# haowenz/FEM

Measured on AMD Instinct MI355X. Metric: mapped Mreads/s (100 bp, e=3) at 1/2/4/8 MI355X + achieved HBM GB/s vs roofline, higher is better.
Workload: dtype u32/u64 integer + 32-bit Myers bit-vectors

## Files before the change

fem_amd/csrc/fem_seed_join.hip.h:

```cpp
#pragma once
#include "fem_seed_dense.hip.h"

namespace femk {

#ifndef FEM_JOIN_SLOTS_HI
#define FEM_JOIN_SLOTS_HI 32768u
#endif
#ifndef FEM_JOIN_OPT
#define FEM_JOIN_OPT 15
#endif
#ifndef FEM_JOIN_OPT_HI
#define FEM_JOIN_OPT_HI 12
#endif
#ifndef FEM_JOIN_ABL
#define FEM_JOIN_ABL 0
#endif
#ifndef FEM_JOIN_SLOTS_LO
#define FEM_JOIN_SLOTS_LO 32768u
#endif
constexpr uint32_t join_slots(int R, bool padded = false) { return R >= 7 ? FEM_JOIN_SLOTS_HI : padded ? FEM_JOIN_SLOTS_LO : 32768u; }
#ifndef FEM_JOIN_BATCH_HI
#define FEM_JOIN_BATCH_HI 3
#endif

#ifndef FEM_JOIN_SPLIT_MAX_R
#define FEM_JOIN_SPLIT_MAX_R 10
#endif
#ifndef FEM_JOIN_BATCH_FULL
#define FEM_JOIN_BATCH_FULL 2
#endif

constexpr uint32_t join_bitmap_words(int R, bool padded = false) { return join_slots(R, padded) / 32u + 4u; }

__device__ __forceinline__ uint32_t lanes_below(uint64_t m) {
  return __builtin_amdgcn_mbcnt_hi((uint32_t)(m >> 32), __builtin_amdgcn_mbcnt_lo((uint32_t)m, 0u));
}

__device__ __forceinline__ void lds_or(uint32_t *w, uint32_t bits) {
  (void)__hip_atomic_fetch_or(w, bits, __ATOMIC_RELAXED, __HIP_MEMORY_SCOPE_WAVEFRONT);
}

template <int R, bool BANKED = false, bool PADDED = false>
__device__ bool join_read(const SeedParams &p, uint32_t s_start, uint32_t s_lo, uint32_t s_freq, uint32_t *bitmap,
                          uint32_t *flg , uint32_t *scatter ,
                          uint32_t *cand_lds, uint32_t &kept0, uint32_t &kept1, uint32_t seq_base = 0u ) {
  const uint32_t ln = lane_id();
  constexpr uint32_t kSlots = join_slots(R, PADDED);
  constexpr uint32_t kSlotBits = kSlots == 65536u ? 16u : kSlots == 32768u ? 15u : 14u;
  static_assert(kSlots == (1u << kSlotBits), "a power of two of slots: 16, 32 or 64 Ki");
  constexpr uint32_t kWordBits = kSlotBits - 5u;
  constexpr uint32_t kWords = kSlots / 32u;
  constexpr uint32_t kPeriodBits = kSlotBits + 3u;
  constexpr uint32_t kFlagCap = dense_flag_cap(R);
  constexpr int kOpt = R <= 6 ? FEM_JOIN_OPT : FEM_JOIN_OPT_HI;
  constexpr bool kOptPairs = (kOpt & 1) != 0, kOptSent = (kOpt & 2) != 0 || (PADDED && R <= 6), kOptLong = (kOpt & 4) != 0, kOptHit = (kOpt & 8) != 0;
  constexpr bool kSecondProbe = true;
  constexpr uint32_t kProbeMin = kOptPairs ? 16u : 8u;
  constexpr uint32_t kFlgStride = kFlagCap + 1u;
  constexpr uint32_t kUnits = 2u * (uint32_t)kStep;
  const uint32_t e = (uint32_t)p.e;
  const uint32_t *occ32 = p.occ32;
  kept0 = 0, kept1 = 0;
  if (__builtin_amdgcn_ballot_w64(s_freq > kDenseMaxList)) return false;
  auto pack_sf = [&](uint32_t start, uint32_t freq) -> uint32_t {
    const uint32_t f_c = freq < (uint32_t)kWave ? freq : (uint32_t)kWave;
    return start | (freq << 16) | ((f_c - (freq != 0u ? 1u : 0u)) << 26);
  };
  const uint32_t s_sf = pack_sf(s_start, s_freq);
  const uint64_t s_addr = (uint64_t)(uintptr_t)(occ32 + s_lo);
  const uint32_t s_alo = (uint32_t)s_addr, s_ahi = (uint32_t)(s_addr >> 32);
  uint32_t lane4 = ln * 4u;
  if (PADDED) asm("" : "+v"(lane4));
  const uint32_t sent_a = 0xF0000000u + ln * 2304u, sent_b = 0xF0000000u + 149504u + (ln << 8);
  static_assert(PADDED || (64u * 2304u + 2048u == 149504u && 149504u + 64u * 256u + 2048u < (1u << kPeriodBits)), "sentinel families inside one period");
  const uint64_t q_is1 = __builtin_amdgcn_ballot_w64((ln >> 2) == 1u), q_is2 = __builtin_amdgcn_ballot_w64((ln >> 2) == 2u),
                 q_is3 = __builtin_amdgcn_ballot_w64((ln >> 2) == 3u);
  uint32_t nxt[R], nxt_sf[R];
  typedef const __attribute__((address_space(1))) uint8_t *GlobalBytes;
  auto run_base_of = [&](uint32_t alo, uint32_t ahi, uint32_t lane) -> GlobalBytes {
    const uint64_t a = (uint64_t)(uint32_t)__builtin_amdgcn_readlane((int)alo, (int)lane) |
                       ((uint64_t)(uint32_t)__builtin_amdgcn_readlane((int)ahi, (int)lane) << 32);
    return (GlobalBytes)(uintptr_t)a;
  };
  auto run_base = [&](uint32_t lane) -> GlobalBytes { return run_base_of(s_alo, s_ahi, lane); };
  auto prefetch_of = [&](uint32_t sf, uint32_t alo, uint32_t ahi, uint32_t u) {
    GlobalBytes base[R];
#pragma unroll
    for (int t = 0; t < R; ++t) {
      nxt_sf[t] = (uint32_t)__builtin_amdgcn_readlane((int)sf, (int)(u * R + t));
      base[t] = run_base_of(alo, ahi, u * R + t);
    }
    if (PADDED) asm volatile("" : "+v"(lane4));
#pragma unroll
    for (int t = 0; t < R; ++t) {
      const uint32_t last4 = nxt_sf[t] >> 24;
      if (PADDED)
        nxt[t] = *(const __attribute__((address_space(1))) uint32_t *)(base[t] + lane4);
      else
        nxt[t] = *(const __attribute__((address_space(1))) uint32_t *)(base[t] + (lane4 < last4 ? lane4 : last4));
    }
  };
  auto prefetch = [&](uint32_t u) { prefetch_of(s_sf, s_alo, s_ahi, u); };
  auto insert = [&](uint32_t v) -> uint32_t {
    const bool valid = v < kDenseVLimit;
    const uint32_t bit = valid ? 1u << ((v >> 3) & 31u) : 0u;
    const uint32_t widx = valid ? __builtin_amdgcn_ubfe(v, 8u, kWordBits) : ln;
    return lds_or_rtn(bitmap + widx, bit) & bit;
  };
  auto word_of = [&](uint32_t x, uint32_t from) -> uint32_t * {
    uint32_t idx = __builtin_amdgcn_ubfe(x, from, kWordBits);
    asm("" : "+v"(idx));
    return bitmap + idx;
  };
  auto insert_plain = [&](uint32_t v) -> uint32_t {
    const uint32_t bit = 1u << ((v >> 3) & 31u);
    return lds_or_rtn(word_of(v, 8u), bit) & bit;
  };
  auto mark = [&](uint32_t v, uint32_t hit) {
    if (FEM_JOIN_ABL & 4) {
      asm volatile("" ::"v"(hit));
      return;
    }
    if (hit) {
      const uint32_t qm = (v >> 3) - 1u, qp = (v >> 3) + 1u;
      lds_or(word_of(qm, 5u), 1u << (qm & 31u));
      lds_or(word_of(qp, 5u), 1u << (qp & 31u));
    }
  };
  auto window = [&](uint32_t v) -> uint32_t {
    const uint32_t qm = (v >> 3) - 1u;
    const uint32_t *w = word_of(qm, 5u);
    return __builtin_amdgcn_alignbit(w[1], w[0], qm & 31u);
  };
  constexpr uint32_t kNearTop = 0x60000000u;
  auto window_top = [&](uint32_t v) -> uint32_t {
    const uint32_t qs = (v >> 3) - 30u;
    const uint32_t *w = word_of(qs, 5u);
    return __builtin_amdgcn_alignbit(w[1], w[0], qs & 31u);
  };
  prefetch(0);
  uint32_t cmin = 0xFFFFFFFFu, cmax = 0u;
  uint32_t surv_groups = 0;
  bool any_hi = false;
#pragma unroll 1
  for (uint32_t u = 0; u < kUnits; ++u) {
    const uint32_t g = u >= (uint32_t)kStep ? u - (uint32_t)kStep : u;
    uint32_t f[R], st[R];
    uint32_t n_g = 0, f_max = 0;
    auto smax = [](uint32_t a_, uint32_t b_) -> uint32_t {
      uint32_t m;
      asm("s_max_u32 %0, %1, %2" : "=s"(m) : "s"(a_), "s"(b_) : "scc");
      return m;
    };
    const bool keep_all = BANKED && (nxt_sf[R - 1] & kSelKeepAll) != 0u;
#pragma unroll
    for (int t = 0; t < R; ++t) {
      const uint32_t sf = nxt_sf[t];
      f[t] = (sf >> 16) & 0xFFu, st[t] = sf & (BANKED ? kSelKeepAll - 1u : 0xFFFFu);
      n_g += f[t];
      f_max = t == 0 ? f[0] : smax(f[t], f_max);
    }
    uint32_t val[R];
#pragma unroll
    for (int t = 0; t < R; ++t) val[t] = nxt[t];
    if (u + 1u < kUnits) prefetch(u + 1u);
    const bool skip = (FEM_JOIN_ABL & 32) || n_g <= (uint32_t)p.a || (n_g == f[R - 1] && !keep_all);
    uint32_t n_flag = 0;
    uint32_t *flg_g = flg + g * kFlgStride;
    if (kOptPairs) {
      flg_g[ln] = 0xFFFFFFFFu;
      if (kFlagCap > (uint32_t)kWave) flg_g[ln + (uint32_t)kWave] = 0xFFFFFFFFu;
    }
    if (!skip) {
      uint32_t first_max = val[0];
#pragma unroll
      for (int t = 1; t < R; ++t) first_max = val[t] > first_max ? val[t] : first_max;
      const bool plain = f_max <= (uint32_t)kWave && __builtin_amdgcn_ballot_w64(first_max >= kDenseRemap) == 0;
      if (R <= FEM_JOIN_SPLIT_MAX_R && plain) {
#define FEM_JOIN_UNIT_PLAIN true
#include "fem_seed_join_unit.hip.h"
#undef FEM_JOIN_UNIT_PLAIN
      } else {
#define FEM_JOIN_UNIT_PLAIN false
#include "fem_seed_join_unit.hip.h"
#undef FEM_JOIN_UNIT_PLAIN
      }
    }
    if (kSecondProbe && n_flag > kProbeMin) {
      const bool have0 = ln < n_flag, have1 = ln + (uint32_t)kWave < n_flag;
      const uint32_t v0 = have0 ? flg_g[ln] : 0u, v1 = have1 ? flg_g[ln + (uint32_t)kWave] : 0u;
      auto key2 = [&](uint32_t v) -> uint32_t {
        const uint32_t slot2 = (__builtin_amdgcn_ubfe(v, 3u, kSlotBits) + (v >> kPeriodBits) * 0x9E5u) & (kSlots - 1u);
        return (slot2 << 3) | (v & 7u);
      };
      auto edge = [&](uint32_t v) -> bool {
        const uint32_t lo = v & ((1u << kPeriodBits) - 1u);
        return lo < e || lo + e >= (1u << kPeriodBits);
      };
      auto wipe = [&](uint32_t k) {
        const uint32_t qm = (k >> 3) - 1u;
        uint32_t *w = bitmap + __builtin_amdgcn_ubfe(qm, 5u, kWordBits);
        w[0] = 0u, w[1] = 0u;
      };
      const uint32_t k0 = key2(v0), k1 = key2(v1);
      const uint32_t h0 = insert(have0 ? k0 : kDenseSent), h1 = insert(have1 ? k1 : kDenseSent);
      if (__builtin_amdgcn_ballot_w64((h0 | h1) != 0u)) mark(k0, h0), mark(k1, h1);
      wave_sync_lds();
      const bool keep0 = have0 && (edge(v0) || (window(k0) & 5u) != 0u);
      const bool keep1 = have1 && (edge(v1) || (window(k1) & 5u) != 0u);
      wave_sync_lds();
      if (have0) wipe(k0);
      if (have1) wipe(k1);
      wave_sync_lds();
      if (ln == 0) bitmap[kWords] = 0xFFFFFFFFu;
      const uint64_t m0 = __builtin_amdgcn_ballot_w64(keep0), m1 = __builtin_amdgcn_ballot_w64(keep1);
      const uint32_t c0 = (uint32_t)__popcll(m0);
      if (keep0) flg_g[__builtin_amdgcn_mbcnt_hi((uint32_t)(m0 >> 32), __builtin_amdgcn_mbcnt_lo((uint32_t)m0, 0u))] = v0;
      if (keep1) flg_g[__builtin_amdgcn_mbcnt_hi((uint32_t)(m1 >> 32), __builtin_amdgcn_mbcnt_lo((uint32_t)m1, c0))] = v1;
      n_flag = c0 + (uint32_t)__popcll(m1);
      wave_sync_lds();
      if (kOptPairs) {
        if (ln >= n_flag) flg_g[ln] = 0xFFFFFFFFu;
        if (kFlagCap > (uint32_t)kWave && ln + (uint32_t)kWave >= n_flag) flg_g[ln + (uint32_t)kWave] = 0xFFFFFFFFu;
        wave_sync_lds();
      }
    }
    if (!(FEM_JOIN_ABL & 2) && n_flag > (uint32_t)p.a) {
      const bool have = ln < n_flag;
      uint32_t fv;
      uint32_t cnt = 0;
      bool pass_hi = false;
      uint32_t fv_hi = 0;
      if (kOptPairs && n_flag <= 8u) {
        const uint32_t xj = flg_g[ln & 7u], fi = flg_g[ln >> 3];
        const uint64_t m = __builtin_amdgcn_ballot_w64(xj - fi <= e);
        cnt = (uint32_t)__popc((uint32_t)(m >> (8u * (ln & 7u))) & 0xFFu);
        fv = have ? xj : 0u;
      } else if (kOptPairs && n_flag <= 16u) {
        const uint32_t xj = flg_g[ln & 15u];
        const uint32_t *fp = flg_g + (ln >> 4);
        const uint64_t m0 = __builtin_amdgcn_ballot_w64(xj - fp[0] <= e), m1 = __builtin_amdgcn_ballot_w64(xj - fp[4] <= e);
        const uint64_t m2 = __builtin_amdgcn_ballot_w64(xj - fp[8] <= e), m3 = __builtin_amdgcn_ballot_w64(xj - fp[12] <= e);
        uint32_t sh16;
        asm volatile("v_lshlrev_b32 %0, 4, %1" : "=v"(sh16) : "v"(ln & 3u));
        const uint32_t r0 = (uint32_t)(m0 >> sh16), r1 = (uint32_t)(m1 >> sh16), r2 = (uint32_t)(m2 >> sh16), r3 = (uint32_t)(m3 >> sh16);
        uint32_t row = r0;
        asm("v_cndmask_b32 %0, %0, %1, %2" : "+v"(row) : "v"(r1), "s"(q_is1));
        asm("v_cndmask_b32 %0, %0, %1, %2" : "+v"(row) : "v"(r2), "s"(q_is2));
        asm("v_cndmask_b32 %0, %0, %1, %2" : "+v"(row) : "v"(r3), "s"(q_is3));
        cnt = (uint32_t)__popc(row & 0xFFFFu);
        fv = have ? xj : 0u;
      } else {
        fv = have ? flg_g[ln] : 0u;
        const uint32_t n_lo = n_flag < (uint32_t)kWave ? n_flag : (uint32_t)kWave;
        if (kFlagCap > (uint32_t)kWave && n_flag > (uint32_t)kWave) {
          const bool have_hi = ln + (uint32_t)kWave < n_flag;
          fv_hi = have_hi ? flg_g[ln + (uint32_t)kWave] : 0u;
          uint32_t cnt_hi = 0;
          for (uint32_t j = 0; j < n_lo; ++j) {
            const uint32_t x = (uint32_t)__builtin_amdgcn_readlane((int)fv, (int)j);
            cnt += (uint32_t)(x - fv <= e), cnt_hi += (uint32_t)(x - fv_hi <= e);
          }
          for (uint32_t j = (uint32_t)kWave; j < n_flag; ++j) {
            const uint32_t x = (uint32_t)__builtin_amdgcn_readlane((int)fv_hi, (int)(j - (uint32_t)kWave));
            cnt += (uint32_t)(x - fv <= e), cnt_hi += (uint32_t)(x - fv_hi <= e);
          }
          pass_hi = have_hi && cnt_hi > (uint32_t)p.a;
        } else {
          for (uint32_t j = 0; j < n_lo; ++j) {
            const uint32_t x = (uint32_t)__builtin_amdgcn_readlane((int)fv, (int)j);
            cnt += (uint32_t)(x - fv <= e);
          }
        }
      }
      const bool pass = have && cnt > (uint32_t)p.a;
      const uint64_t pm = __builtin_amdgcn_ballot_w64(pass);
      if (__builtin_amdgcn_ballot_w64(pass_hi)) {
        any_hi = true;
        cmin = pass_hi && fv_hi < cmin ? fv_hi : cmin;
        cmax = pass_hi && fv_hi > cmax ? fv_hi : cmax;
      }
      if (pm != 0) {
        surv_groups |= 1u << g;
        if (ln == 0) {
          scatter[4u * g] = (uint32_t)pm, scatter[4u * g + 1u] = (uint32_t)(pm >> 32);
          scatter[4u * g + 2u] = n_flag;
        }
        cmin = pass && fv < cmin ? fv : cmin;
        cmax = pass && fv > cmax ? fv : cmax;
      }
    }
    if (g != (uint32_t)kStep - 1u) continue;
    uint32_t kept = 0, cv = 0;
    if (surv_groups != 0 || any_hi) {
      const uint32_t lo_all = wave_min_u32(cmin), hi_all = wave_max_u32(cmax);
      if (hi_all - lo_all <= e) {
        cv = ln == 0 ? lo_all : 0u;
        kept = 1;
      } else if (any_hi) {
        return false;
      } else {
        wave_sync_lds();
        const uint32_t surv = scatter[ln];
#pragma unroll 1
        for (uint32_t gg = 0; gg < (uint32_t)kStep; ++gg) {
          if (!((surv_groups >> gg) & 1u)) continue;
          const uint64_t pm = (uint64_t)(uint32_t)__builtin_amdgcn_readlane((int)surv, (int)(4u * gg)) |
                              ((uint64_t)(uint32_t)__builtin_amdgcn_readlane((int)surv, (int)(4u * gg + 1u)) << 32);
          const uint32_t nfl = (uint32_t)__builtin_amdgcn_readlane((int)surv, (int)(4u * gg + 2u));
          const uint32_t nF = (uint32_t)__popcll(pm);
          const bool mine = (pm >> ln) & 1ull;
          const uint32_t fv = ln < nfl ? flg[gg * kFlgStride + ln] : 0u;
          uint32_t rank = 0;
          for (uint64_t m = pm; m;) {
            const int j = __builtin_ctzll(m);
            m &= m - 1;
            const uint32_t x = (uint32_t)__builtin_amdgcn_readlane((int)fv, j);
            rank += (uint32_t)(x < fv || (x == fv && (uint32_t)j < ln));
          }
          wave_sync_lds();
          if (mine) scatter[rank] = fv;
          wave_sync_lds();
          const uint32_t fs = ln < nF ? scatter[ln] : 0u;
          kept = dense_merge_group(cv, kept, fs, nF, e);
          if (kept == 0xFFFFFFFFu) return false;
        }
      }
    }
    cand_lds[(u >= (uint32_t)kStep ? (uint32_t)kWave : 0u) + ln] = cv;
    if (u >= (uint32_t)kStep) kept1 = kept; else kept0 = kept;
    cmin = 0xFFFFFFFFu, cmax = 0u, any_hi = false;
    surv_groups = 0;
  }
  return true;
}

#ifndef FEM_JOIN_WAVES_LO
#define FEM_JOIN_WAVES_LO 7
#endif
#ifndef FEM_JOIN_WAVES_HI
#define FEM_JOIN_WAVES_HI 6
#endif

constexpr int join_waves(int R) { return R <= 6 ? FEM_JOIN_WAVES_LO : FEM_JOIN_WAVES_HI; }

template <int R, bool BANKED = false, bool PADDED = false>
__device__ __forceinline__ void seed_join_body(const SeedParams &p, uint8_t *smem) {
  constexpr uint32_t kSeeds = (uint32_t)(kStep * R);
  static_assert(2 * kStep * R <= kWave, "both strands' seeds must fit the lanes of one wave");
  const uint32_t ln = lane_id();
  const uint32_t wave_in_block = (uint32_t)__builtin_amdgcn_readfirstlane((int)(threadIdx.x >> 6));
  uint8_t *wbase = smem + (size_t)wave_in_block * p.lay.wave_bytes;
  uint32_t *scatter = (uint32_t *)(wbase + p.lay.X);
  uint32_t *flg = (uint32_t *)(wbase + p.lay.A);
  uint32_t *bitmap = (uint32_t *)(wbase + p.lay.F);
  uint2 *blk_entries = (uint2 *)(wbase + p.lay.B);
  uint32_t *cand_lds = (uint32_t *)(wbase + p.lay.sf);
  uint2 *seqtab = (uint2 *)(smem + p.lay.picked);
  const bool small_ref = p.n_seq <= (uint32_t)kWave;
  if (wave_in_block == 0) seqtab[ln] = ln < p.n_seq ? make_uint2(p.goff[ln], p.seq_len[ln]) : make_uint2(0xFFFFFFFFu, 0u);
  __syncthreads();
  for (uint32_t i = ln; i < join_bitmap_words(R, PADDED); i += kWave) bitmap[i] = i < join_slots(R, PADDED) / 32u ? 0u : 0xFFFFFFFFu;
  wave_sync_lds();
  unsigned long long pre_sum = 0, cand_sum = 0;
  SlotChunk chunk, qchunk;

  auto queue_slow = [&](uint32_t read) {
    if (qchunk.left == 0) {
      uint32_t base = 0;
      if (ln == 0) base = atomicAdd(&p.ctr[2], kQueueChunk);
      qchunk.next = bcast0(base);
      qchunk.left = kQueueChunk;
    }
    if (qchunk.next < p.slow_cap) {
      if (ln == 0) p.slow_queue[qchunk.next] = read;
    } else if (ln == 0) {
      atomicOr(&p.ctr[1], kFlagQueueOverflow);
    }
    ++qchunk.next, --qchunk.left;
  };

  for (;;) {
    uint32_t pull = 0;
    if (ln == 0) pull = atomicAdd(p.work_cursor, kReadBlock);
    pull = bcast0(pull);
    if (p.read_begin >= p.n_reads || pull >= p.n_reads - p.read_begin) break;
    const uint32_t r0 = p.read_begin + pull;
    const uint32_t n_blk = p.n_reads - r0 < kReadBlock ? p.n_reads - r0 : kReadBlock;
    if (ln < 2u * kReadBlock) blk_entries[ln] = make_uint2(kBlkSkip, 0u);
    uint2 hdr = make_uint2(kSelSlow, 0u);
    if (ln < n_blk) hdr = p.sel_hdr[r0 + ln];
    uint2 sel_next = make_uint2(0u, 0u);
    auto sel_of = [&](uint32_t read) -> uint2 {
      typedef const __attribute__((address_space(1))) uint8_t *GlobalBytes;
      uint32_t lane8;
      asm volatile("v_lshlrev_b32 %0, 3, %1" : "=v"(lane8) : "v"(ln));
      const GlobalBytes row = (GlobalBytes)(uintptr_t)(p.sel + (size_t)read * (2u * kSeeds));
      const uint64_t w = *(const __attribute__((address_space(1))) uint64_t *)(row + lane8);
      return make_uint2((uint32_t)w, (uint32_t)(w >> 32));
    };
    if (!BANKED && ln < 2u * kSeeds) sel_next = sel_of(r0);
    for (uint32_t rb = 0; rb < n_blk; ++rb) {
      const uint32_t read = r0 + rb;
      const uint32_t h0 = (uint32_t)__builtin_amdgcn_readlane((int)hdr.x, (int)rb);
      const uint32_t status = h0 & 3u, L = h0 >> 8;
      const uint2 sel = sel_next;
      if (!BANKED && rb + 1u < n_blk && ln < 2u * kSeeds) sel_next = sel_of(read + 1u);
      if (status == kSelSlow) continue;
      if (status == kSelNone) {
        if (ln / 2u == rb) blk_entries[ln] = make_uint2(0u, 0u);
        continue;
      }
      if constexpr (BANKED) {
        constexpr uint32_t kStash = (uint32_t)kWave;
        uint64_t *stash = (uint64_t *)(wbase + p.lay.gq);
        uint32_t acc[2] = {0u, 0u};
        bool failed = false;
        for (uint32_t b = 0; b < p.n_banks && !failed; ++b) {
          uint2 sel_b = make_uint2(0u, 0u);
          if (ln < 2u * kSeeds) sel_b = p.sel[((size_t)read * p.n_banks + b) * (2u * kSeeds) + ln];
          uint32_t kept0 = 0, kept1 = 0;
          if (!join_read<R, true>(p, sel_b.y & 0xFFFFu, sel_b.x, sel_b.y >> 16, bitmap, flg, scatter, cand_lds, kept0, kept1, p.bank_first[b])) {
            failed = true;
            break;
          }
          const uint32_t sq_lo = p.bank_first[b], sq_hi = p.bank_first[b + 1u];
#pragma unroll 1
          for (uint32_t strand = 0; strand < 2u; ++strand) {
            const uint32_t kept = strand ? kept1 : kept0;
            if (kept == 0) continue;
            const uint32_t v = cand_lds[strand * (uint32_t)kWave + ln];
            uint32_t sq = 0, pos = 0, slen = 0;
            if (small_ref) {
              const uint2 tab = seqtab[ln];
              const bool mine = ln >= sq_lo && ln < sq_hi;
              for (uint32_t i = 0; i < kept; ++i) {
                const uint32_t vi = (uint32_t)__builtin_amdgcn_readlane((int)v, (int)i);
                const uint32_t s_i = sq_lo + (uint32_t)__popcll(__builtin_amdgcn_ballot_w64(mine && tab.x <= vi)) - 1u;
                const uint32_t g_i = (uint32_t)__builtin_amdgcn_readlane((int)tab.x, (int)s_i);
                const uint32_t l_i = (uint32_t)__builtin_amdgcn_readlane((int)tab.y, (int)s_i);
                if (ln == i) sq = s_i, pos = vi - g_i, slen = l_i;
              }
            } else if (ln < kept) {
              sq = p.blkseq[(size_t)b * p.blk_stride + (v >> kDenseBlkShift)];
              while (sq + 1u < sq_hi && p.goff[sq + 1u] <= v) ++sq;
              pos = v - p.goff[sq];
              slen = p.seq_len[sq];
            }
            const bool ok = ln < kept && pos >= (uint32_t)p.e && pos + L + (uint32_t)p.e < slen;
            const uint64_t mo = __ballot(ok);
            const uint32_t n_ok = (uint32_t)__popcll(mo);
            if (acc[strand] + n_ok > kStash) {
              failed = true;
              break;
            }
            if (ok) stash[strand * kStash + acc[strand] + lanes_below(mo)] = (((uint64_t)sq << 32) | pos) - (uint64_t)p.e;
            acc[strand] += n_ok;
          }
        }
        if (failed) {
          queue_slow(read);
          continue;
        }
        pre_sum += (uint32_t)__builtin_amdgcn_readlane((int)hdr.y, (int)rb);
        wave_sync_lds();
#pragma unroll 1
        for (uint32_t strand = 0; strand < 2u; ++strand) {
          const uint32_t n_out = acc[strand];
          uint32_t base = 0;
          if (n_out > 0) {
            if (n_out <= chunk.left) {
              base = chunk.next;
              chunk.next += n_out, chunk.left -= n_out;
            } else {
              pad_chunk(p, chunk);
              if (ln == 0) base = atomicAdd(&p.ctr[0], kSlotChunk);
              base = bcast0(base);
              chunk.next = base + n_out, chunk.left = kSlotChunk - n_out;
            }
            if (n_out > p.cand_cap || base > p.cand_cap - n_out) {
              if (ln == 0) atomicOr(&p.ctr[1], kFlagCandOverflow);
            } else {
              for (uint32_t i = ln; i < n_out; i += (uint32_t)kWave) {
                p.cand[base + i] = stash[strand * kStash + i];
                p.cand_meta[base + i] = (read * 2u + strand) | (i < (n_out & ~7u) ? kMeta16 : 0u);
              }
            }
          }
          if (ln == 0) blk_entries[2u * rb + strand] = make_uint2(base, n_out);
          cand_sum += n_out;
        }
        wave_sync_lds();
        continue;
      }
      const uint32_t s_lo = sel.x, s_start = sel.y & 0xFFFFu, s_freq = sel.y >> 16;
      uint32_t kept0 = 0, kept1 = 0;
      if (!join_read<R, false, PADDED>(p, s_start, s_lo, s_freq, bitmap, flg, scatter, cand_lds, kept0, kept1)) {
        queue_slow(read);
        continue;
      }
      if (FEM_JOIN_ABL & 16) kept0 = kept1 = 0;
      pre_sum += (uint32_t)__builtin_amdgcn_readlane((int)hdr.y, (int)rb);
#pragma unroll 1
      for (uint32_t strand = 0; strand < 2u; ++strand) {
        const uint32_t kept = strand ? kept1 : kept0;
        uint64_t out = 0;
        bool ok = false;
        if (kept == 0) {
          if (ln == 0) blk_entries[2u * rb + strand] = make_uint2(0u, 0u);
          continue;
        }
        const uint32_t v = cand_lds[strand * (uint32_t)kWave + ln];
        uint32_t sq = 0, pos = 0, slen = 0;
        if (small_ref) {
          const uint2 tab = seqtab[ln];
          for (uint32_t i = 0; i < kept; ++i) {
            const uint32_t vi = (uint32_t)__builtin_amdgcn_readlane((int)v, (int)i);
            const uint32_t s_i = (uint32_t)__popcll(__builtin_amdgcn_ballot_w64(tab.x <= vi)) - 1u;
            const uint32_t g_i = (uint32_t)__builtin_amdgcn_readlane((int)tab.x, (int)s_i);
            const uint32_t l_i = (uint32_t)__builtin_amdgcn_readlane((int)tab.y, (int)s_i);
            if (ln == i) sq = s_i, pos = vi - g_i, slen = l_i;
          }
        } else if (ln < kept) {
          sq = p.blkseq[v >> kDenseBlkShift];
          while (sq + 1u < p.n_seq && p.goff[sq + 1u] <= v) ++sq;
          pos = v - p.goff[sq];
          slen = p.seq_len[sq];
        }
        if (ln < kept) {
          ok = pos >= (uint32_t)p.e && pos + L + (uint32_t)p.e < slen;
          out = (((uint64_t)sq << 32) | pos) - (uint64_t)p.e;
        }
        const uint64_t mo = __ballot(ok);
        const uint32_t n_out = (uint32_t)__popcll(mo);
        uint32_t base = 0;
        if (n_out > 0) {
          if (n_out <= chunk.left) {
            base = chunk.next;
            chunk.next += n_out, chunk.left -= n_out;
          } else {
            pad_chunk(p, chunk);
            if (ln == 0) base = atomicAdd(&p.ctr[0], kSlotChunk);
            base = bcast0(base);
            chunk.next = base + n_out, chunk.left = kSlotChunk - n_out;
          }
          if (n_out > p.cand_cap || base > p.cand_cap - n_out) {
            if (ln == 0) atomicOr(&p.ctr[1], kFlagCandOverflow);
          } else if (ok) {
            const uint32_t rank = lanes_below(mo), at = base + rank;
            p.cand[at] = out;
            p.cand_meta[at] = (read * 2u + strand) | (rank < (n_out & ~7u) ? kMeta16 : 0u);
          }
        }
        if (ln == 0) blk_entries[2u * rb + strand] = make_uint2(base, n_out);
        cand_sum += n_out;
      }
    }
    wave_sync_lds();
    const uint2 entry = blk_entries[ln];
    wave_sync_lds();
    if (ln < 2u * kReadBlock && r0 + ln / 2u < p.n_reads && entry.x != kBlkSkip) {
      __builtin_nontemporal_store(entry.x, &p.cand_begin[r0 * 2u + ln]);
      __builtin_nontemporal_store(entry.y, &p.cand_count[r0 * 2u + ln]);
    }
  }
  pad_chunk(p, chunk);
  for (uint32_t i = ln; i < qchunk.left; i += kWave)
    if (qchunk.next + i < p.slow_cap) p.slow_queue[qchunk.next + i] = kInvalidRead;
  if (ln == 0) {
    if (pre_sum) atomicAdd(&p.stats[0], pre_sum);
    if (cand_sum) atomicAdd(&p.stats[1], cand_sum);
  }
}


#define FEM_JOIN_KERNEL(R, WAVES)                                                                                               \
  __global__ void __launch_bounds__(256) __attribute__((amdgpu_waves_per_eu(WAVES, 8))) seed_join_kernel_r##R(SeedParams p) {                         \
    extern __shared__ __attribute__((aligned(16))) uint8_t smem[];                                                               \
    seed_join_body<R>(p, smem);                                                                                                  \
  }                                                                                                                              \
  __global__ void __launch_bounds__(256) __attribute__((amdgpu_waves_per_eu(FEM_JOIN_WAVES_HI, 8))) seed_join_banked_kernel_r##R(SeedParams p) {  \
    extern __shared__ __attribute__((aligned(16))) uint8_t smem[];                                                               \
    seed_join_body<R, true>(p, smem);                                                                                            \
  }                                                                                                                              \
  __global__ void __launch_bounds__(256) __attribute__((amdgpu_waves_per_eu(WAVES, 8))) seed_join_kernel_padded_r##R(SeedParams p) {  \
    extern __shared__ __attribute__((aligned(16))) uint8_t smem[];                                                               \
    seed_join_body<R, false, true>(p, smem);                                                                                     \
  }
FEM_JOIN_KERNEL(1, FEM_JOIN_WAVES_LO)
FEM_JOIN_KERNEL(2, FEM_JOIN_WAVES_LO)
FEM_JOIN_KERNEL(3, FEM_JOIN_WAVES_LO)
FEM_JOIN_KERNEL(4, FEM_JOIN_WAVES_LO)
FEM_JOIN_KERNEL(5, FEM_JOIN_WAVES_LO)
FEM_JOIN_KERNEL(6, FEM_JOIN_WAVES_LO)
FEM_JOIN_KERNEL(7, FEM_JOIN_WAVES_HI)
FEM_JOIN_KERNEL(8, FEM_JOIN_WAVES_HI)
FEM_JOIN_KERNEL(9, FEM_JOIN_WAVES_HI)
FEM_JOIN_KERNEL(10, FEM_JOIN_WAVES_HI)
#undef FEM_JOIN_KERNEL

}
```

fem_amd/csrc/fem_seed_join_unit.hip.h:

```cpp
#ifndef FEM_JOIN_UNIT_PLAIN
#error "fem_seed_join_unit.hip.h is a part of join_read (fem_seed_join.hip.h): define FEM_JOIN_UNIT_PLAIN true or false and include it there"
#endif
      constexpr bool kPlain = FEM_JOIN_UNIT_PLAIN;
      const bool long_lists = !kPlain && f_max > (uint32_t)kWave;
      uint32_t hv[R];
#pragma unroll
      for (int t = 0; t < R; ++t) hv[t] = kDenseSent;
      if (long_lists) {
#pragma unroll
        for (int t = 0; t < R; ++t) {
          if (kOptLong && f[t] <= (uint32_t)kWave) continue;
          const uint32_t last4 = f[t] > (uint32_t)kWave ? (f[t] - 1u) * 4u : 0u;
          const uint32_t at4 = lane4 + 4u * (uint32_t)kWave;
          if (PADDED)
            hv[t] = *(const __attribute__((address_space(1))) uint32_t *)(run_base(u * R + t) + at4);
          else
            hv[t] = *(const __attribute__((address_space(1))) uint32_t *)(run_base(u * R + t) + (at4 < last4 ? at4 : last4));
        }
      }
      bool remap = false;
      if (!kPlain) {
        uint32_t raw_max = val[0];
#pragma unroll
        for (int t = 1; t < R; ++t) raw_max = val[t] > raw_max ? val[t] : raw_max;
        if (long_lists) {
#pragma unroll
          for (int t = 0; t < R; ++t) raw_max = hv[t] > raw_max ? hv[t] : raw_max;
        }
        remap = __builtin_amdgcn_ballot_w64(raw_max >= kDenseRemap) != 0;
      }
      uint32_t max_u = 0;
      bool any_u = true;
      uint64_t vm[R];
#pragma unroll
      for (int t = 0; t < R; ++t) vm[t] = 0;
      if (__builtin_expect(remap, 0)) {
        uint32_t mx = 0, have_u = 0;
        auto settle = [&](uint32_t &v, bool have, uint32_t start) {
          const uint32_t raw = v;
          v = kDenseSent;
          if (have) {
            v = raw - start;
            if (raw >= kDenseRemap) {
              const uint32_t sq = (raw - kDenseRemap) >> 10, pos = raw & (kDenseNear - 1u);
              v = pos >= start ? p.goff[seq_base + sq] + pos - start : kDenseSent;
            }
          }
        };
#pragma unroll 1
        for (int t = 0; t < R; ++t) {
          uint32_t a_ = 0, b_ = 0;
#pragma unroll
          for (int q = 0; q < R; ++q) a_ = q == t ? val[q] : a_, b_ = q == t ? hv[q] : b_;
          uint32_t f_t = 0, st_t = 0;
#pragma unroll
          for (int q = 0; q < R; ++q) f_t = q == t ? f[q] : f_t, st_t = q == t ? st[q] : st_t;
          settle(a_, ln < f_t, st_t);
          settle(b_, long_lists && ln + (uint32_t)kWave < f_t, st_t);
          if (t < R - 1) {
            if (a_ < kDenseVLimit) mx = a_ > mx ? a_ : mx, have_u = 1;
            if (b_ < kDenseVLimit) mx = b_ > mx ? b_ : mx, have_u = 1;
          }
          if (kOptSent) a_ = a_ < kDenseVLimit ? a_ : sent_b;
#pragma unroll
          for (int q = 0; q < R; ++q) val[q] = q == t ? a_ : val[q], hv[q] = q == t ? b_ : hv[q];
        }
        any_u = __builtin_amdgcn_ballot_w64(have_u != 0) != 0;
        max_u = wave_max_u32(mx);
        if (kOptSent) {
#pragma unroll
          for (int t = 0; t < R; ++t) vm[t] = __builtin_amdgcn_ballot_w64(val[t] < kDenseVLimit);
        }
      } else {
        if (kOptSent) {
#pragma unroll
          for (int t = 0; t < R; ++t) {
            if (PADDED) {
              vm[t] = __builtin_amdgcn_ballot_w64(ln < f[t]);
              val[t] -= st[t];
            } else {
              const bool in = ln < f[t];
              vm[t] = __builtin_amdgcn_ballot_w64(in);
              val[t] = (in ? val[t] : sent_a) - st[t];
            }
          }
        } else {
#pragma unroll
          for (int t = 0; t < R; ++t) val[t] = PADDED ? val[t] - st[t] : ln < f[t] ? val[t] - st[t] : kDenseSent;
        }
        if (long_lists) {
#pragma unroll
          for (int t = 0; t < R; ++t) {
            if (PADDED && (!kOptLong || f[t] > (uint32_t)kWave))
              hv[t] -= st[t];
            else
              hv[t] = ln + (uint32_t)kWave < f[t] ? hv[t] - st[t] : kDenseSent;
          }
#pragma unroll
          for (int t = 0; t < R - 1; ++t) {
            const uint32_t l_lo = (uint32_t)__builtin_amdgcn_readlane((int)val[t], (int)((f[t] - 1u) & 63u));
            const uint32_t l_hi = (uint32_t)__builtin_amdgcn_readlane((int)hv[t], (int)((f[t] - 65u) & 63u));
            const uint32_t lastv = f[t] > (uint32_t)kWave ? l_hi : l_lo;
            max_u = f[t] && lastv > max_u ? lastv : max_u;
          }
        } else {
#pragma unroll
          for (int t = 0; t < R - 1; ++t) {
            const uint32_t lastv = (uint32_t)__builtin_amdgcn_readlane((int)val[t], (int)((f[t] - 1u) & 63u));
            max_u = f[t] && lastv > max_u ? lastv : max_u;
          }
        }
      }
      if (keep_all) any_u = true, max_u = 0xFFFFFFFFu;
      if (any_u) {
        if (kOptSent) {
          const bool keep = val[R - 1] <= max_u;
          vm[R - 1] &= __builtin_amdgcn_ballot_w64(keep);
          val[R - 1] = keep ? val[R - 1] : sent_b;
        } else {
          val[R - 1] = val[R - 1] <= max_u ? val[R - 1] : kDenseSent;
        }
        if (long_lists) hv[R - 1] = hv[R - 1] <= max_u ? hv[R - 1] : kDenseSent;
        constexpr int kBatch = R > 6 ? FEM_JOIN_BATCH_HI : kPlain ? R : FEM_JOIN_BATCH_FULL < R ? FEM_JOIN_BATCH_FULL : R;
        auto flag_chunk = [&](uint32_t v, uint32_t xw, uint64_t valid, bool exact) {
          if (FEM_JOIN_ABL & 1) {
            asm volatile("" ::"v"(xw), "v"(v));
            return;
          }
          bool near = xw >= kNearTop;
          if (exact) near = near && v < kDenseVLimit;
          const uint64_t m = exact ? __builtin_amdgcn_ballot_w64(near) : __builtin_amdgcn_ballot_w64(near) & valid;
          if (!exact && m == 0) return;
          uint32_t pos = __builtin_amdgcn_mbcnt_hi((uint32_t)(m >> 32), __builtin_amdgcn_mbcnt_lo((uint32_t)m, n_flag));
          pos = pos < kFlagCap ? pos : kFlagCap;
          if (near) flg_g[pos] = v;
          n_flag += (uint32_t)__popcll(m);
        };
        auto insert_all = [&](uint32_t (&vals)[R], bool checked, bool second) {
#pragma unroll
          for (int t0 = 0; t0 < R; t0 += kBatch) {
            uint32_t hit[kBatch];
#pragma unroll
            for (int q = 0; q < kBatch; ++q)
              if (t0 + q < R) {
                hit[q] = 0;
                if (second && kOptLong && f[t0 + q] <= (uint32_t)kWave) continue;
                hit[q] = checked ? insert(vals[t0 + q]) : insert_plain(vals[t0 + q]);
              }
#pragma unroll
            for (int q = 0; q < kBatch; ++q)
              if (t0 + q < R) {
                if (second && kOptLong && f[t0 + q] <= (uint32_t)kWave) continue;
                if (kOptHit) {
                  mark(vals[t0 + q], hit[q]);
                } else if (__builtin_amdgcn_ballot_w64(hit[q] != 0u)) {
                  mark(vals[t0 + q], hit[q]);
                }
              }
          }
        };
        auto flag_all = [&](uint32_t (&vals)[R], bool second, bool exact) {
#pragma unroll
          for (int t0 = 0; t0 < R; t0 += kBatch) {
            uint32_t x[kBatch];
#pragma unroll
            for (int q = 0; q < kBatch; ++q)
              if (t0 + q < R) {
                if (second && kOptLong && f[t0 + q] <= (uint32_t)kWave) continue;
                x[q] = window_top(vals[t0 + q]);
              }
#pragma unroll
            for (int q = 0; q < kBatch; ++q)
              if (t0 + q < R) {
                if (second && kOptLong && f[t0 + q] <= (uint32_t)kWave) continue;
                flag_chunk(vals[t0 + q], x[q], vm[t0 + q], exact);
              }
          }
        };
        if (FEM_JOIN_ABL & 64) {
#pragma unroll
          for (int t = 0; t < R; ++t) asm volatile("" ::"v"(val[t]), "v"(hv[t]));
        } else {
        insert_all(val, !kOptSent, false);
        if (long_lists) insert_all(hv, true, true);
        wave_sync_lds();
        if (!kOptSent || __builtin_expect(remap, 0)) flag_all(val, false, true); else flag_all(val, false, false);
        if (long_lists) flag_all(hv, true, true);
        wave_sync_lds();
        }
        if (!(FEM_JOIN_ABL & 8)) {
          uint4 *b4 = (uint4 *)bitmap;
#pragma unroll
          for (uint32_t k = 0; k < kWords / 4u / (uint32_t)kWave; ++k) b4[k * (uint32_t)kWave + ln] = make_uint4(0u, 0u, 0u, 0u);
        }
        wave_sync_lds();
        if (n_flag > kFlagCap) return false;
      }
```

Baseline: 379.4.

## Batch flag appends, drop validity ballots, and mark neighbors in the hit word

Raises the default join option mask for R<=6 to turn on three paths. Neighbour marks go into the word already returned by the insert atomic, so only edge bits need a second LDS atomic. In the sentinel path, near-flag appends are batched per lane across chunks and written with one ballot/mbcnt flush instead of one per chunk. The per-list validity-mask ballots are skipped. This cuts LDS atomics and wave-wide ballot work, but relies on sentinel values never being flagged, so a mistaken sentinel could change which candidates are kept.

After: 393.2, median of 6. 3.6% higher.

```diff
diff --git a/fem_amd/csrc/fem_seed_join.hip.h b/fem_amd/csrc/fem_seed_join.hip.h
--- a/fem_amd/csrc/fem_seed_join.hip.h
+++ b/fem_amd/csrc/fem_seed_join.hip.h
@@ -7,7 +7,7 @@
 #define FEM_JOIN_SLOTS_HI 32768u
 #endif
 #ifndef FEM_JOIN_OPT
-#define FEM_JOIN_OPT 15
+#define FEM_JOIN_OPT 127
 #endif
 #ifndef FEM_JOIN_OPT_HI
 #define FEM_JOIN_OPT_HI 12
@@ -54,6 +54,7 @@
   constexpr uint32_t kFlagCap = dense_flag_cap(R);
   constexpr int kOpt = R <= 6 ? FEM_JOIN_OPT : FEM_JOIN_OPT_HI;
   constexpr bool kOptPairs = (kOpt & 1) != 0, kOptSent = (kOpt & 2) != 0 || (PADDED && R <= 6), kOptLong = (kOpt & 4) != 0, kOptHit = (kOpt & 8) != 0;
+  constexpr bool kOptOnce = (kOpt & 16) != 0 && kOptSent, kOptNoMask = (kOpt & 32) != 0 && kOptOnce, kOptOwn = (kOpt & 64) != 0;
   constexpr bool kSecondProbe = true;
   constexpr uint32_t kProbeMin = kOptPairs ? 16u : 8u;
   constexpr uint32_t kFlgStride = kFlagCap + 1u;
@@ -101,30 +102,41 @@
     }
   };
   auto prefetch = [&](uint32_t u) { prefetch_of(s_sf, s_alo, s_ahi, u); };
-  auto insert = [&](uint32_t v) -> uint32_t {
+  typedef __attribute__((address_space(3))) uint32_t *LdsWord;
+  auto insert = [&](uint32_t v, LdsWord &w) -> uint32_t {
     const bool valid = v < kDenseVLimit;
     const uint32_t bit = valid ? 1u << ((v >> 3) & 31u) : 0u;
     const uint32_t widx = valid ? __builtin_amdgcn_ubfe(v, 8u, kWordBits) : ln;
-    return lds_or_rtn(bitmap + widx, bit) & bit;
+    w = (LdsWord)(bitmap + widx);
+    return lds_or_rtn((uint32_t *)w, bit) & bit;
   };
   auto word_of = [&](uint32_t x, uint32_t from) -> uint32_t * {
     uint32_t idx = __builtin_amdgcn_ubfe(x, from, kWordBits);
     asm("" : "+v"(idx));
     return bitmap + idx;
   };
-  auto insert_plain = [&](uint32_t v) -> uint32_t {
+  auto insert_plain = [&](uint32_t v, LdsWord &w) -> uint32_t {
     const uint32_t bit = 1u << ((v >> 3) & 31u);
-    return lds_or_rtn(word_of(v, 8u), bit) & bit;
-  };
-  auto mark = [&](uint32_t v, uint32_t hit) {
+    w = (LdsWord)word_of(v, 8u);
+    return lds_or_rtn((uint32_t *)w, bit) & bit;
+  };
+  auto mark = [&](uint32_t v, uint32_t hit, LdsWord w) {
     if (FEM_JOIN_ABL & 4) {
       asm volatile("" ::"v"(hit));
       return;
     }
     if (hit) {
-      const uint32_t qm = (v >> 3) - 1u, qp = (v >> 3) + 1u;
-      lds_or(word_of(qm, 5u), 1u << (qm & 31u));
-      lds_or(word_of(qp, 5u), 1u << (qp & 31u));
+      if (kOptOwn) {
+        lds_or((uint32_t *)w, (hit << 1) | (hit >> 1));
+        if (hit & 0x80000001u) {
+          const uint32_t q = (hit >> 31) != 0u ? (v >> 3) + 1u : (v >> 3) - 1u;
+          lds_or(word_of(q, 5u), 1u << (q & 31u));
+        }
+      } else {
+        const uint32_t qm = (v >> 3) - 1u, qp = (v >> 3) + 1u;
+        lds_or(word_of(qm, 5u), 1u << (qm & 31u));
+        lds_or(word_of(qp, 5u), 1u << (qp & 31u));
+      }
     }
   };
   auto window = [&](uint32_t v) -> uint32_t {
@@ -203,8 +215,9 @@
         w[0] = 0u, w[1] = 0u;
       };
       const uint32_t k0 = key2(v0), k1 = key2(v1);
-      const uint32_t h0 = insert(have0 ? k0 : kDenseSent), h1 = insert(have1 ? k1 : kDenseSent);
-      if (__builtin_amdgcn_ballot_w64((h0 | h1) != 0u)) mark(k0, h0), mark(k1, h1);
+      LdsWord w0, w1;
+      const uint32_t h0 = insert(have0 ? k0 : kDenseSent, w0), h1 = insert(have1 ? k1 : kDenseSent, w1);
+      if (__builtin_amdgcn_ballot_w64((h0 | h1) != 0u)) mark(k0, h0, w0), mark(k1, h1, w1);
       wave_sync_lds();
       const bool keep0 = have0 && (edge(v0) || (window(k0) & 5u) != 0u);
       const bool keep1 = have1 && (edge(v1) || (window(k1) & 5u) != 0u);
diff --git a/fem_amd/csrc/fem_seed_join_unit.hip.h b/fem_amd/csrc/fem_seed_join_unit.hip.h
--- a/fem_amd/csrc/fem_seed_join_unit.hip.h
+++ b/fem_amd/csrc/fem_seed_join_unit.hip.h
@@ -67,7 +67,7 @@
         }
         any_u = __builtin_amdgcn_ballot_w64(have_u != 0) != 0;
         max_u = wave_max_u32(mx);
-        if (kOptSent) {
+        if (kOptSent && !kOptNoMask) {
 #pragma unroll
           for (int t = 0; t < R; ++t) vm[t] = __builtin_amdgcn_ballot_w64(val[t] < kDenseVLimit);
         }
@@ -76,11 +76,11 @@
 #pragma unroll
           for (int t = 0; t < R; ++t) {
             if (PADDED) {
-              vm[t] = __builtin_amdgcn_ballot_w64(ln < f[t]);
+              if (!kOptNoMask) vm[t] = __builtin_amdgcn_ballot_w64(ln < f[t]);
               val[t] -= st[t];
             } else {
               const bool in = ln < f[t];
-              vm[t] = __builtin_amdgcn_ballot_w64(in);
+              if (!kOptNoMask) vm[t] = __builtin_amdgcn_ballot_w64(in);
               val[t] = (in ? val[t] : sent_a) - st[t];
             }
           }
@@ -115,16 +115,37 @@
       if (any_u) {
         if (kOptSent) {
           const bool keep = val[R - 1] <= max_u;
-          vm[R - 1] &= __builtin_amdgcn_ballot_w64(keep);
+          if (!kOptNoMask) vm[R - 1] &= __builtin_amdgcn_ballot_w64(keep);
           val[R - 1] = keep ? val[R - 1] : sent_b;
         } else {
           val[R - 1] = val[R - 1] <= max_u ? val[R - 1] : kDenseSent;
         }
         if (long_lists) hv[R - 1] = hv[R - 1] <= max_u ? hv[R - 1] : kDenseSent;
         constexpr int kBatch = R > 6 ? FEM_JOIN_BATCH_HI : kPlain ? R : FEM_JOIN_BATCH_FULL < R ? FEM_JOIN_BATCH_FULL : R;
+        uint32_t fl = 0xFFFFFFFFu;
+        uint64_t acc = 0;
+        auto flush = [&]() {
+          const bool ok = fl < kDenseVLimit;
+          const uint64_t m = __builtin_amdgcn_ballot_w64(ok);
+          uint32_t pos = __builtin_amdgcn_mbcnt_hi((uint32_t)(m >> 32), __builtin_amdgcn_mbcnt_lo((uint32_t)m, n_flag));
+          pos = pos < kFlagCap ? pos : kFlagCap;
+          if (ok) flg_g[pos] = fl;
+          n_flag += (uint32_t)__popcll(m);
+          fl = 0xFFFFFFFFu;
+          acc = 0;
+        };
         auto flag_chunk = [&](uint32_t v, uint32_t xw, uint64_t valid, bool exact) {
           if (FEM_JOIN_ABL & 1) {
             asm volatile("" ::"v"(xw), "v"(v));
+            return;
+          }
+          if (kOptOnce && !exact) {
+            const bool near_ = xw >= kNearTop;
+            const uint64_t m = __builtin_amdgcn_ballot_w64(near_);
+            if ((kOptNoMask ? m : m & valid) == 0) return;
+            if ((m & acc) != 0) flush();
+            fl = near_ ? v : fl;
+            acc |= m;
             return;
           }
           bool near = xw >= kNearTop;
@@ -140,21 +161,22 @@
 #pragma unroll
           for (int t0 = 0; t0 < R; t0 += kBatch) {
             uint32_t hit[kBatch];
+            LdsWord hw[kBatch];
 #pragma unroll
             for (int q = 0; q < kBatch; ++q)
               if (t0 + q < R) {
                 hit[q] = 0;
                 if (second && kOptLong && f[t0 + q] <= (uint32_t)kWave) continue;
-                hit[q] = checked ? insert(vals[t0 + q]) : insert_plain(vals[t0 + q]);
+                hit[q] = checked ? insert(vals[t0 + q], hw[q]) : insert_plain(vals[t0 + q], hw[q]);
               }
 #pragma unroll
             for (int q = 0; q < kBatch; ++q)
               if (t0 + q < R) {
                 if (second && kOptLong && f[t0 + q] <= (uint32_t)kWave) continue;
                 if (kOptHit) {
-                  mark(vals[t0 + q], hit[q]);
+                  mark(vals[t0 + q], hit[q], hw[q]);
                 } else if (__builtin_amdgcn_ballot_w64(hit[q] != 0u)) {
-                  mark(vals[t0 + q], hit[q]);
+                  mark(vals[t0 + q], hit[q], hw[q]);
                 }
               }
           }
@@ -176,6 +198,7 @@
                 flag_chunk(vals[t0 + q], x[q], vm[t0 + q], exact);
               }
           }
+          if (kOptOnce && !exact && acc != 0) flush();
         };
         if (FEM_JOIN_ABL & 64) {
 #pragma unroll
```
